# tatsy/opengl-raytracer

Measured on AMD Instinct MI355X. Metric: Mrays/s at 1920x1080, 8 bounces, higher is better.
Workload: dtype f32

## Files before the change

### opengl-raytracer_amd/csrc/pt_kernel.hip.h

```cpp
#pragma once
#include <hip/hip_runtime.h>
#include <stdint.h>

#include <type_traits>
#include "trav_asm.hip.h"
#include "scan_asm.hip.h"
#include "texture.hip.h"
#include "maps.hip.h"
#include "environment.hip.h"

namespace glrtx {

constexpr int kBlockThreads = 256;
constexpr int kTile = 16;
constexpr int REF_ABSENT = INT32_MIN;
constexpr int REF_FIN = INT32_MIN;
constexpr int kMaxLdsMaterials = 256;
constexpr int kMaxLdsLights = 64;
constexpr int kTopForks = 128;

constexpr float PT_EPS = 1.0e-4f;
constexpr float PT_INFTY = 1.0e8f;
constexpr float PT_PI = 3.14159274101257324f;
constexpr float PT_2PI = 6.28318548202514648f;
// ... 486 lines not shown
    }
    asm volatile(
        "s_mov_b64 %[entry], exec\n\t"
        "s_mov_b64 %[act], exec\n\t"
        GLRTX_ASM_SET_VBASE
        "v_bfrev_b32 v[GLRTX_VB+11], 1\n\t"
        GLRTX_REP(GLRTX_STEPS_PER_TRIP, GLRTX_TRAV_STEP_ASM_LANE)
        "99:\n\t"
        "s_mov_b64 exec, %[entry]"
        : [th] "+&v"(T.h.t), [tri] "+&v"(T.h.tri), [hu] "+&v"(T.h.u), [hv] "+&v"(T.h.v), [cur] "+&v"(T.cur), [sp] "+&v"(T.sp),
          [entry] "=&s"(s_entry), [act] "=&s"(s_act), [leaf] "=&s"(s_leaf), [bl] "=&s"(s_bl), [br] "=&s"(s_br), [pop] "=&s"(s_pop), [tmp] "=&s"(s_tmp) GLRTX_TS_OPERANDS
        : [ox] "v"(T.ox), [oy] "v"(T.oy), [oz] "v"(T.oz), [dx] "v"(T.dx), [dy] "v"(T.dy), [dz] "v"(T.dz), [ix] "v"(T.ix), [iy] "v"(T.iy), [iz] "v"(T.iz),
          [sd] "v"(T.stop_d), [stk] "v"(stk), [base] "s"(sc.nodes0), [bias] "s"(sc.node_bias), [eps] "s"(PT_EPS)
        : "vcc", "scc", "memory", GLRTX_ASM_VCLOBBERS GLRTX_TS_CLOBBERS);
}

struct TravLoop {
    unsigned long long act, uns;
    int pos, cnt;
    unsigned flags;
    unsigned rid, nr;
    float4 co, cd;
    float ix, iy, iz, lim;
};
#define GLRTX_LOOP_OUT \
    [th] "+&v"(T.h.t), [tri] "+&v"(T.h.tri), [hu] "+&v"(T.h.u), [hv] "+&v"(T.h.v), [cur] "+&v"(T.cur), [sp] "+&v"(T.sp), \
    [ox] "+&v"(T.ox), [oy] "+&v"(T.oy), [oz] "+&v"(T.oz), [dx] "+&v"(T.dx), [dy] "+&v"(T.dy), [dz] "+&v"(T.dz), [ix] "+&v"(T.ix), [iy] "+&v"(T.iy), [iz] "+&v"(T.iz), \
    [sd] "+&v"(T.stop_d), [rid] "+&v"(L.rid), [nr] "+&v"(L.nr), [act] "+&s"(L.act), [uns] "+&s"(L.uns), [pos] "+&s"(L.pos), \
    [entry] "=&s"(s_entry), [was] "=&s"(s_was), [leaf] "=&s"(s_leaf), [bl] "=&s"(s_bl), [br] "=&s"(s_br), [pop] "=&s"(s_pop), [tmp] "=&s"(s_tmp), \
    [n] "=&s"(s_n), [take] "=&s"(s_take), [why] "=&s"(why)
#define GLRTX_LOOP_IN \
    [cox] "v"(L.co.x), [coy] "v"(L.co.y), [coz] "v"(L.co.z), [cow] "v"(L.co.w), [cdx] "v"(L.cd.x), [cdy] "v"(L.cd.y), [cdz] "v"(L.cd.z), [cdw] "v"(L.cd.w), \
    [cix] "v"(L.ix), [ciy] "v"(L.iy), [ciz] "v"(L.iz), [clim] "v"(L.lim), [stk] "v"(stk), [cnt] "s"(cnt), [flags] "s"(flags), [rmin] "s"(rmin), [smax] "s"(smax), \
    [hbase] "s"(hbase), [lb] "s"(lb), [eps] "s"(PT_EPS)
template <int FETCH>
DEV int trav_loop_asm(const DevScene &sc, int *stack, Trav &T, TravLoop &L, int rmin, int smax, const void *hbase, unsigned lb, unsigned rk) {
    unsigned long long s_entry, s_was, s_leaf, s_bl, s_br, s_pop, s_tmp;
    int s_n, s_take, why;
    const unsigned stk = (unsigned)(uintptr_t)stack;
    static_assert(kBlockThreads * 8 == 1 << 11 && REF_FIN == INT32_MIN, "see trav_steps_asm");
    const int cnt = __builtin_amdgcn_readfirstlane(L.cnt);
    const unsigned flags = (unsigned)__builtin_amdgcn_readfirstlane((int)L.flags);
    rmin = __builtin_amdgcn_readfirstlane(rmin);
    smax = __builtin_amdgcn_readfirstlane(smax);
    const unsigned par16 = (threadIdx.x & 1u) << 4;
    const unsigned bias_e = sc.node_bias + par16, bias_o = sc.node_bias + 16u - par16;
    if constexpr ((FETCH & kWgwfCompact) != 0) {
        static_assert((FETCH & ~kWgwfCompact) == 0, "the compact layout has the one-record-per-lane fetch only");
        asm volatile(GLRTX_TRAV_LOOP_ASM(GLRTX_REP(GLRTX_STEPS_PER_TRIP, GLRTX_TRAV_STEP_ASM_COMPACT), "v[GLRTX_VB+22]", "0")
                     : GLRTX_LOOP_OUT
                     : GLRTX_LOOP_IN, [cbase] "s"(sc.cnodes), [rk] "s"(rk)
                     : "vcc", "scc", "memory", GLRTX_ASM_VCLOBBERS_COMPACT);
    } else if constexpr (FETCH == 2) {
        asm volatile(GLRTX_TRAV_LOOP_ASM(GLRTX_REP(GLRTX_STEPS_PER_TRIP_HALF, GLRTX_TRAV_STEP_ASM_PAIR GLRTX_TRAV_STEP_ASM_LANE), "v[GLRTX_VB+11]", "%[root]")
                     : GLRTX_LOOP_OUT
                     : GLRTX_LOOP_IN, [root] "s"(sc.root_ref), [base] "s"(sc.nodes0), [bias] "s"(sc.node_bias), [odd] "s"(0xAAAAAAAAAAAAAAAAull), [biase] "v"(bias_e), [biaso] "v"(bias_o)
                     : "vcc", "scc", "memory", GLRTX_ASM_VCLOBBERS_PAIR);
    } else if constexpr (FETCH == 1) {
        asm volatile(GLRTX_TRAV_LOOP_ASM(GLRTX_REP(GLRTX_STEPS_PER_TRIP, GLRTX_TRAV_STEP_ASM_PAIR), "v[GLRTX_VB+11]", "%[root]")
                     : GLRTX_LOOP_OUT
                     : GLRTX_LOOP_IN, [root] "s"(sc.root_ref), [base] "s"(sc.nodes0), [odd] "s"(0xAAAAAAAAAAAAAAAAull), [biase] "v"(bias_e), [biaso] "v"(bias_o)
                     : "vcc", "scc", "memory", GLRTX_ASM_VCLOBBERS_PAIR);
    } else {
        static_assert(FETCH == 0, "node fetch: 0 lane, 1 pair, 2 alternating, kWgwfCompact");
        asm volatile(GLRTX_TRAV_LOOP_ASM(GLRTX_REP(GLRTX_STEPS_PER_TRIP, GLRTX_TRAV_STEP_ASM_LANE), "v[GLRTX_VB+11]", "%[root]")
                     : GLRTX_LOOP_OUT
                     : GLRTX_LOOP_IN, [root] "s"(sc.root_ref), [base] "s"(sc.nodes0), [bias] "s"(sc.node_bias)
                     : "vcc", "scc", "memory", GLRTX_ASM_VCLOBBERS);
    }
    (void)rk; (void)bias_e; (void)bias_o;
    return why;
}

template <bool CLOSEST>
DEV void tri_test(Hit &h, int t, float ox, float oy, float oz, float dx, float dy, float dz, float v0x, float v0y, float v0z, float e1x,
                  float e1y, float e1z, float e2x, float e2y, float e2z, float tmin = PT_EPS) {
    const float tx = ox - v0x, ty = oy - v0y, tz = oz - v0z;
    const float px = dy * e2z - dz * e2y;
    const float py = dz * e2x - dx * e2z;
    const float pz = dx * e2y - dy * e2x;
    const float det = dot3(e1x, e1y, e1z, px, py, pz);
    const float U = dot3(tx, ty, tz, px, py, pz);
    const float inv = rcp_newton(det);
    const float u = U * inv;
    const bool ok_u = !(-PT_EPS < det && det < PT_EPS) && !(u < 0.0f || 1.0f < u);
    if (!__any(ok_u)) return;
    const float qx = ty * e1z - tz * e1y;
    const float qy = tz * e1x - tx * e1z;
    const float qz = tx * e1y - ty * e1x;
    const float V = dot3(dx, dy, dz, qx, qy, qz);
    const float v = V * inv;
    const bool ok_v = ok_u && !(v < 0.0f || 1.0f < inv * (U + V));
    if (!__any(ok_v)) return;
    const float tt = dot3(e2x, e2y, e2z, qx, qy, qz) * inv;
    const bool hit = ok_v && !(tmin >= tt);
// ... 1443 lines not shown
#define GLRTX_PRIO_SHADE 0
#endif
#ifndef GLRTX_WGWF_WAVES
#define GLRTX_WGWF_WAVES 4
#endif

#ifdef GLRTX_PHASE_STATS
__device__ unsigned long long g_phase_cycles[8];
__device__ uint4 g_trip_log[16][64];
#define PH_STAMP(var) const unsigned long long var = __builtin_amdgcn_s_memtime()
#define PH_ADD(i, t0, t1) do { if (threadIdx.x == 0) atomicAdd(&g_phase_cycles[i], (t1) - (t0)); } while (0)
#else
#define PH_STAMP(var)
#define PH_ADD(i, t0, t1)
#endif

#ifdef GLRTX_RAY_LOG
struct RayLog { float4 *rays; uint2 *trips; unsigned long long cap_rays; unsigned cap_trips; unsigned on; };
__device__ RayLog g_ray_log;
__device__ unsigned long long g_ray_log_n;
__device__ unsigned g_ray_log_trips;
#endif

DEV int wgwf_suspend_max();

#if defined(GLRTX_CXX_STEP) || defined(GLRTX_TRAV_STATS) || defined(GLRTX_PHASE_STATS) || defined(GLRTX_STEP_TIMING) || defined(GLRTX_RAY_LOG) || defined(GLRTX_CXX_LOOP)
#define GLRTX_TRAV_LOOP_CXX
#endif
template <bool VINE, int FETCH>
DEV void wg_traverse_phase(const KernelArgs &a, const WfArgs &w, const float4 *root, int *stack, const float4 *rq, int n_rays,
                           unsigned *ray_head, unsigned *light_bits, unsigned long long &rays, float4 *suspend_area) {
    const int lane = threadIdx.x & 63;
    const uint2 *ranks = reinterpret_cast<const uint2 *>(light_bits + kWgPathsMax / 32);
    if (VINE) {
        for (;;) {
            int base = 0;
            if (lane == 0) base = (int)atomicAdd(ray_head, 64u);
            base = __builtin_amdgcn_readfirstlane(base);
            if (base >= n_rays) break;
            float4 o = make_float4(0.f, 0.f, 0.f, __uint_as_float(WF_INVALID)), d = o;
            if (base + lane < n_rays) { o = ld_stream(&rq[2 * (size_t)(base + lane)]); d = ld_stream(&rq[2 * (size_t)(base + lane) + 1]); }
            const unsigned r = __float_as_uint(o.w);
            const bool shadow = (r & 1u) != 0u;
            const Hit h = trav_scan<true>(a.sc, o.x, o.y, o.z, d.x, d.y, d.z, r != WF_INVALID, shadow ? shadow_limit(d.w, a.sc.shadow_limited) : PT_INFTY,
                                          shadow ? d.w : -__builtin_inff());
            if (r != WF_INVALID) {
                rays++;
                if (r & 1u) { if (nee_accepted(d.w, h.t, h.tri >= 0)) atomicOr(&light_bits[r >> 6], 1u << ((r >> 1) & 31u)); }
                else st_stream(w.H(r >> 1), make_float4(h.t, __int_as_float(h.tri), h.u, h.v));
            }
        }
        return;
    }
    [[maybe_unused]] const unsigned long long lt_mask = (1ull << lane) - 1ull;
    const float4 none = make_float4(0.f, 0.f, 0.f, __uint_as_float(WF_INVALID));
    float4 cur_o = none, cur_d = none;
    float cur_ix = 0.f, cur_iy = 0.f, cur_iz = 0.f;
    [[maybe_unused]] int cur_pos = 0;
    int cur_cnt = 0;
#ifndef GLRTX_TRAV_LOOP_CXX
    float cur_lim = PT_INFTY;
#endif
    auto fetch = [&](float4 &o, float4 &d) -> int {
        int base = 0;
        if (lane == 0) base = (int)atomicAdd(ray_head, 64u);
        base = __builtin_amdgcn_readfirstlane(base);
        int cnt = n_rays - base;
        cnt = cnt < 0 ? 0 : (cnt > 64 ? 64 : cnt);
        if (lane < cnt) {
            o = ld_stream(&rq[2 * (size_t)(base + lane)]);
            d = ld_stream(&rq[2 * (size_t)(base + lane) + 1]);
            cur_ix = frcp(d.x); cur_iy = frcp(d.y); cur_iz = frcp(d.z);
            const bool shadow = (__float_as_uint(o.w) & 1u) != 0u;
            float t0;
            if (a.sc.root_boxed && !box_pass(root[0], root[1], o.x, o.y, o.z, cur_ix, cur_iy, cur_iz, shadow ? shadow_limit(d.w, a.sc.shadow_limited) : PT_INFTY, t0))
                d.w = __uint_as_float(__float_as_uint(d.w) | 0x80000000u);
#ifndef GLRTX_TRAV_LOOP_CXX
            cur_lim = shadow ? shadow_limit(__builtin_fabsf(d.w), a.sc.shadow_limited) : PT_INFTY;
#endif
        }
        return cnt;
    };
    cur_cnt = fetch(cur_o, cur_d);
    bool exhausted = cur_cnt == 0;
    const bool fetched_any = cur_cnt > 0;
    bool active = false;
    bool unsaved = false;
    unsigned rid = 0;
    Trav T;
    T.cur = 0; T.sp = 0;
    T.h.t = PT_INFTY; T.h.tri = -1; T.h.u = 0.f; T.h.v = 0.f;
#ifdef GLRTX_STEP_TIMING
    StepTiming step_timing;
#endif
    float4 *const susp = suspend_area + (size_t)kSuspendF4 * threadIdx.x;
    {
        const float4 s3 = susp[3];
        if (s3.z != 0.0f) {
            const float4 s0 = susp[0], s1 = susp[1], s2 = susp[2];
            susp[3] = make_float4(0.f, 0.f, 0.f, 0.f);
            T.ox = s0.x; T.oy = s0.y; T.oz = s0.z;
            rid = __float_as_uint(w.H(__float_as_uint(s0.w) >> 1)->y);
// ... 11 lines not shown
#ifdef GLRTX_FAULT_INJECT
            if (fault_dropped) active = false;
#endif
        }
    }
    auto save_hit = [&]() {
        const unsigned id = rid >> 1;
        if (rid & 1u) {
            if (nee_accepted(T.stop_d, T.h.t, T.h.tri >= 0)) atomicOr(&light_bits[id >> 5], 1u << (id & 31u));
        } else *w.H(id) = make_float4(T.h.t, __int_as_float(T.h.tri), T.h.u, T.h.v);
        unsaved = false;
    };
#ifndef GLRTX_TRAV_LOOP_CXX
    static_assert(WF_INVALID == 0xFFFFFFFFu, "trav_asm.hip.h compares a ray id with the inline constant -1");
    {
        TravLoop L;
        L.act = __ballot(active); L.uns = 0ull;
        L.pos = 0; L.cnt = cur_cnt;
        L.flags = exhausted ? 1u : 0u;
        L.rid = rid; L.nr = 0u;
        const void *const hbase = w.H(0u);
        const unsigned lb = (unsigned)(uintptr_t)light_bits;
        const int smax = wgwf_suspend_max();
        int why;
        for (;;) {
            L.co = cur_o; L.cd = cur_d; L.ix = cur_ix; L.iy = cur_iy; L.iz = cur_iz; L.lim = cur_lim;
            why = trav_loop_asm<FETCH>(a.sc, stack, T, L, w.refill_min, smax, hbase, lb, (unsigned)(uintptr_t)ranks);
            if (why != 1) break;
            cur_cnt = cur_cnt == 64 ? fetch(cur_o, cur_d) : 0;
            L.pos = 0; L.cnt = cur_cnt;
            L.flags = cur_cnt == 0 ? (1u | 2u | (fetched_any ? 4u : 0u)) : 2u;
        }
        rid = L.rid;
        rays += L.nr;
        active = ((L.act >> lane) & 1ull) != 0ull;
        unsaved = ((L.uns >> lane) & 1ull) != 0ull;
        if (why == 2 && active) {
            susp[0] = make_float4(T.ox, T.oy, T.oz, __uint_as_float(rid));
            susp[1] = make_float4(T.dx, T.dy, T.dz, T.stop_d);
            susp[2] = make_float4(T.h.t, __int_as_float(T.h.tri), T.h.u, T.h.v);
            susp[3] = make_float4(__int_as_float(T.cur), __int_as_float(T.sp), 1.0f, 0.f);
            float mark = kHitSuspended, zero = 0.f;
            asm volatile("" : "+v"(mark), "+v"(zero));
            *w.H(rid >> 1) = make_float4(mark, zero, zero, zero);
            active = false;
        }
    }
#else
#ifdef GLRTX_PHASE_STATS
    unsigned long long ph_refill = 0ull, ph_refills = 0ull, ph_step = 0ull;
#endif
    for (;;) {
        unsigned long long idle = __ballot(!active);
        if ((int)__popcll(idle) >= w.refill_min || idle == ~0ull) {
#ifdef GLRTX_PHASE_STATS
            const unsigned long long rf0 = __builtin_amdgcn_s_memtime();
#endif
            while (idle != 0ull && !exhausted) {
                if (cur_pos >= cur_cnt) {
                    cur_cnt = cur_cnt == 64 ? fetch(cur_o, cur_d) : 0;
                    cur_pos = 0;
                    if (cur_cnt == 0) { exhausted = true; break; }
                }
                const int n = __popcll(idle);
                const int avail = cur_cnt - cur_pos;
                const int take = n < avail ? n : avail;
                const int rank = __popcll(idle & lt_mask);
                const int src = (cur_pos + rank) & 63;
                const float ox = __shfl(cur_o.x, src), oy = __shfl(cur_o.y, src), oz = __shfl(cur_o.z, src);
                const unsigned new_rid = (unsigned)__shfl((int)__float_as_uint(cur_o.w), src);
                const float dx = __shfl(cur_d.x, src), dy = __shfl(cur_d.y, src), dz = __shfl(cur_d.z, src);
                const float dist_m = __shfl(cur_d.w, src);
                const float ix = __shfl(cur_ix, src), iy = __shfl(cur_iy, src), iz = __shfl(cur_iz, src);
                if (!active && rank < take) {
                    if (unsaved) save_hit();
                    rid = new_rid;
                    if (rid != WF_INVALID) {
                        rays++;
                        const bool shadow = (rid & 1u) != 0u;
                        const float dist = __builtin_fabsf(dist_m);
                        T.ox = ox; T.oy = oy; T.oz = oz; T.dx = dx; T.dy = dy; T.dz = dz; T.ix = ix; T.iy = iy; T.iz = iz;
                        T.h.t = shadow ? shadow_limit(dist, a.sc.shadow_limited) : PT_INFTY; T.h.tri = -1; T.h.u = 0.f; T.h.v = 0.f;
                        T.stop_d = shadow ? dist : -__builtin_inff();
                        T.sp = 0;
                        T.cur = (FETCH & kWgwfCompact) ? 0 : a.sc.root_ref;
#ifdef GLRTX_TRAV_STATS
                        T.iters = 0;
#endif
                        active = (__float_as_uint(dist_m) & 0x80000000u) == 0u;
                        unsaved = !active;
                    }
                }
                cur_pos += take;
                idle = __ballot(!active);
            }
#ifdef GLRTX_PHASE_STATS
            ph_refill += __builtin_amdgcn_s_memtime() - rf0; ph_refills += 1ull;
#endif
        }
        if (!__any(active)) {
            if (exhausted) break;
            continue;
        }
        if (exhausted && fetched_any) {
            const unsigned long long ma = __ballot(active);
            const int suspend_max = wgwf_suspend_max();
            if (__ballot(active && (rid & 1u) != 0u) == 0ull && (int)__popcll(ma) <= suspend_max) {
                if (active) {
                    susp[0] = make_float4(T.ox, T.oy, T.oz, __uint_as_float(rid));
                    susp[1] = make_float4(T.dx, T.dy, T.dz, T.stop_d);
                    susp[2] = make_float4(T.h.t, __int_as_float(T.h.tri), T.h.u, T.h.v);
                    susp[3] = make_float4(__int_as_float(T.cur), __int_as_float(T.sp), 1.0f, 0.f);
// ... 301 lines not shown
                unsigned tid = threadIdx.x;
                asm volatile("" : "+v"(tid));
                if (tid < kWgPathsMax / 32) light_bits[tid] = 0u;
            }
            const int nr = (int)ctl[2 + cur], np = (int)ctl[4 + cur];
            float4 *rq_w = rayQ + 2 * ((size_t)cur * 2 * kWgPaths + nr);
            const WgwfKernArgs *kt = wgwf_kernargs();
            const unsigned new_base = kt->w.set_base(cur, (int)blockIdx.x) + (unsigned)np;
            for (int k = threadIdx.x; k < got; k += kBlockThreads) {
                int id = tile0 * 64 + k;
                if (ADAPT) {
                    const int g = tile0 + (k >> 6), n_active = (int)*kt->adapt_count;
                    const int frame = g / n_active;
                    id = frame * kt->w.total + kt->adapt_list[g - frame * n_active] * 64 + (k & 63);
                }
                float4 ro = make_float4(0.f, 0.f, 0.f, __uint_as_float(WF_INVALID)), rd = ro;
                const bool go = wf_generate_one(kt->a, kt->w, lds_cam, id, new_base + (unsigned)k, ro, rd);
                rq_w[2 * k] = ro;
                rq_w[2 * k + 1] = rd;
                (void)go;
            }
            __syncthreads();
            if (tid_topup == 0u) { ctl[2 + cur] = (unsigned)(nr + got); ctl[4 + cur] = (unsigned)(np + got); ctl[1] = 0u; }
        }
        __syncthreads();
        PH_STAMP(pg1);
        PH_ADD(0, pg0, pg1);
        const int n_rays = (int)ctl[2 + cur], n_paths = (int)ctl[4 + cur];
        if (n_paths == 0) {
            if (look_again) continue;
            break;
        }
        const float4 *rq = rayQ + 2 * ((size_t)cur * 2 * kWgPaths);

#ifdef GLRTX_RAY_LOG
        if (g_ray_log.on) {
            if (threadIdx.x == 0) {
                const unsigned long long base = atomicAdd(&g_ray_log_n, (unsigned long long)n_rays);
                ctl[9] = 0u;
                if (base + (unsigned long long)n_rays <= g_ray_log.cap_rays) {
                    const unsigned t = atomicAdd(&g_ray_log_trips, 1u);
                    if (t < g_ray_log.cap_trips) { g_ray_log.trips[t] = make_uint2((unsigned)base, (unsigned)n_rays); ctl[8] = (unsigned)base; ctl[9] = 1u; }
                }
            }
            __syncthreads();
            if (ctl[9]) {
                float4 *dst = g_ray_log.rays + 2 * (size_t)ctl[8];
                for (int i = threadIdx.x; i < 2 * n_rays; i += kBlockThreads) dst[i] = rq[i];
            }
            __syncthreads();
        }
#endif
        PH_STAMP(pt0);
        __builtin_amdgcn_s_setprio(GLRTX_PRIO_TRAVERSE);
        wg_traverse_phase<VINE, NODE_FETCH>(a, w, lds_root, stack, rq, n_rays, &ctl[1], light_bits, rays, rayQ + kWgSuspendAt);
        __builtin_amdgcn_s_setprio(GLRTX_PRIO_SHADE);
        PH_STAMP(pt1);
        __syncthreads();
        PH_STAMP(pt2);
        PH_ADD(1, pt0, pt1);
        PH_ADD(2, pt1, pt2);

        const WgwfKernArgs *ks = wgwf_kernargs();
        wg_shade_phase<VOL, TEX, MAPS>(ks->a, ks->w, lds_mats, lds_cam, light_bits, n_paths, rayQ + 2 * ((size_t)(cur ^ 1) * 2 * kWgPaths),
                            &ctl[2 + (cur ^ 1)], &ctl[4 + (cur ^ 1)], ks->w.set_base(cur, (int)blockIdx.x), ks->w.set_base(cur ^ 1, (int)blockIdx.x), rays, &ctl[10]);
        PH_STAMP(ps1);
        __syncthreads();
        PH_STAMP(ps2);
        PH_ADD(3, pt2, ps1);
        PH_ADD(4, ps1, ps2);
#ifdef GLRTX_PHASE_STATS
        if (threadIdx.x == 0 && (blockIdx.x & 63) == 0 && blockIdx.x / 64 < 16) {
            uint4 *lg = g_trip_log[blockIdx.x / 64];
            const unsigned n = lg[0].x + 1u;
            if (n < 64u) { lg[n] = make_uint4((unsigned)n_rays, (unsigned)n_paths, (unsigned)(pt2 - pt0), (unsigned)(ps2 - pt2)); lg[0].x = n; }
        }
#endif
        unsigned tid_end = threadIdx.x;
// ... 31 lines not shown
__global__ __launch_bounds__(kBlockThreads, GLRTX_WGWF_WAVES) void pt_replay_traverse(const KernelArgs a, const WfArgs w, unsigned *work_counter, float4 *wg_queues,
                                                                                      const float4 *log, const uint2 *trips, int n_trips) {
    extern __shared__ __attribute__((aligned(16))) unsigned char lds_raw[];
    const int mat_f4 = a.sc.lds_head_f4;
    unsigned char *pl = lds_raw + (size_t)mat_f4 * sizeof(float4);
    int *stack = reinterpret_cast<int *>(pl) + 2 * threadIdx.x;
    pl += (size_t)2 * a.sc.stack_entries * kBlockThreads * sizeof(int);
    unsigned *ctl = reinterpret_cast<unsigned *>(pl);
    float4 *lds_root = reinterpret_cast<float4 *>(pl + kWgCtlWords * sizeof(unsigned));
    unsigned *light_bits = reinterpret_cast<unsigned *>(pl + kWgCtlWords * sizeof(unsigned) + 32 + kCamFloatsPadded * 4 + kLdsSeeds * 8);
    if (threadIdx.x == 64) lds_root[0] = a.sc.root_lo;
    if (threadIdx.x == 65) lds_root[1] = a.sc.root_hi;
    float4 *rayQ = wg_queues + (size_t)blockIdx.x * kWgQueueF4;
    rayQ[kWgSuspendAt + (size_t)kSuspendF4 * threadIdx.x + 3] = make_float4(0.f, 0.f, 0.f, 0.f);
    unsigned long long rays = 0;
    __syncthreads();
    for (;;) {
        if (threadIdx.x == 0) { ctl[0] = atomicAdd(work_counter, 1u); ctl[1] = 0u; }
        if (threadIdx.x < kWgPathsMax / 32) light_bits[threadIdx.x] = 0u;
        __syncthreads();
        const unsigned t = ctl[0];
        if (t >= (unsigned)n_trips) break;
        const uint2 tr = trips[t];
        __builtin_amdgcn_s_setprio(GLRTX_PRIO_TRAVERSE);
        wg_traverse_phase<false, FETCH>(a, w, lds_root, stack, log + 2 * (size_t)tr.x, (int)tr.y, &ctl[1], light_bits, rays, rayQ + kWgSuspendAt);
        __builtin_amdgcn_s_setprio(GLRTX_PRIO_SHADE);
        __syncthreads();
    }
    flush_rays<true>(a, rays);
}
#endif


constexpr float kAdaptLumFloor = 1e-3f;
constexpr int kAdaptCompactThreads = 1024;

__global__ __launch_bounds__(256) void adaptive_select_kernel(const float4 *accum, const float4 *half, int pitch_f4, int width, int rows, int tiles8_x, int n_tiles,
                                                              float threshold, int min_samples, unsigned char *mask, float *tile_err) {
    const int tile = blockIdx.x * 4 + (threadIdx.x >> 6), k = threadIdx.x & 63;
    if (tile >= n_tiles) return;
    const int x = (tile % tiles8_x) * 8 + (k & 7), y = (tile / tiles8_x) * 8 + (k >> 3);
    const bool in = x < width && y < rows;
    float d = 0.0f;
    bool force = false;
    if (in) {
        const size_t at = (size_t)y * pitch_f4 + x;
        const float4 c = ld_stream(&accum[at]), h = ld_stream(&half[at]);
        force = c.w < (float)min_samples || h.w == 0.0f;
// ... 136 lines not shown
```

### opengl-raytracer_amd/csrc/trav_asm.hip.h

```cpp
#pragma once

#ifndef GLRTX_STEPS_PER_TRIP
#define GLRTX_STEPS_PER_TRIP 6
#endif
#ifndef GLRTX_ASM_VBASE
#define GLRTX_ASM_VBASE 96
#endif
static_assert(GLRTX_STEPS_PER_TRIP % 2 == 0, "the alternating form of the node fetch unrolls steps in pairs");
#define GLRTX_STEPS_PER_TRIP_HALF_(n) GLRTX_HALF_##n
#define GLRTX_HALF_2 1
#define GLRTX_HALF_4 2
#define GLRTX_HALF_6 3
#define GLRTX_HALF_8 4
#define GLRTX_STEPS_PER_TRIP_HALF_X(n) GLRTX_STEPS_PER_TRIP_HALF_(n)
#define GLRTX_STEPS_PER_TRIP_HALF GLRTX_STEPS_PER_TRIP_HALF_X(GLRTX_STEPS_PER_TRIP)
#define GLRTX_STR_(x) #x
#define GLRTX_STR(x) GLRTX_STR_(x)
#define GLRTX_ASM_SET_VBASE ".set GLRTX_VB, " GLRTX_STR(GLRTX_ASM_VBASE) "\n\t"
#if GLRTX_ASM_VBASE == 96
#define GLRTX_ASM_VCLOBBERS "v96", "v97", "v98", "v99", "v100", "v101", "v102", "v103", "v104", "v105", "v106", "v107", "v108", "v109", "v110", "v111", "v112", "v113", "v114", "v115", "v116", "v117"
#define GLRTX_ASM_VCLOBBERS_PAIR GLRTX_ASM_VCLOBBERS, "v118", "v119"
#define GLRTX_ASM_VCLOBBERS_COMPACT GLRTX_ASM_VCLOBBERS_PAIR
#elif GLRTX_ASM_VBASE == 72
#define GLRTX_ASM_VCLOBBERS "v72", "v73", "v74", "v75", "v76", "v77", "v78", "v79", "v80", "v81", "v82", "v83", "v84", "v85", "v86", "v87", "v88", "v89", "v90", "v91", "v92", "v93"
// ... 340 lines not shown
    "s_or_b64 %[pop], %[pop], vcc\n\t"                                                                                                                \
    "21:\n\t"                                                                                                                                          \
    "s_mov_b64 exec, %[pop]\n\t"                                         \
    "s_cbranch_execz 30f\n\t"                                                                                                                          \
    "10:\n\t"                                                                                                                                          \
    "v_cmp_ne_u32 vcc, 0, %[sp]\n\t"                                                                                                                   \
    "v_cndmask_b32 %[cur], " FIN ", %[cur], vcc\n\t"                                                                \
    "s_and_b64 exec, exec, vcc\n\t"                                                                                                                    \
    "s_cbranch_execz 30f\n\t"                                                                                                                          \
    "v_add_u32 %[sp], -1, %[sp]\n\t"                                                                                                                   \
    "v_lshl_add_u32 v[GLRTX_VB+15], %[sp], 11, %[stk]\n\t"                                                                                                       \
    "ds_read_b64 v[GLRTX_VB+16:GLRTX_VB+17], v[GLRTX_VB+15]\n\t"                                                                                                  \
    "s_waitcnt lgkmcnt(0)\n\t"                                                                                                                         \
    "v_mov_b32 %[cur], v[GLRTX_VB+17]\n\t"                                                                                                                       \
    "v_cmp_gt_f32 vcc, v[GLRTX_VB+16], %[th]\n\t"                                                                                                                \
    "s_and_b64 exec, exec, vcc\n\t"                                                                                                                    \
    "s_cbranch_execnz 10b\n\t"                                                                                                                         \
    "30:\n\t"                                                                                                                                          \
    "s_mov_b64 exec, %[act]\n\t"                                                                                  \
    GLRTX_TS_END                                                                                                                       \
    "v_cmpx_ne_u32_e64 %[act], %[cur], " FIN "\n\t"                                                                             \
    "s_cbranch_execz 99f\n\t"

#define GLRTX_TRAV_LOOP_ASM(STEPS, FIN, ROOT) \
    "s_mov_b64 %[entry], exec\n\t" \
    "s_mov_b64 exec, -1\n\t" \
    GLRTX_ASM_SET_VBASE \
    "v_bfrev_b32 " FIN ", 1\n\t" \
    "s_bitcmp1_b32 %[flags], 1\n\t"                                      \
    "s_cbranch_scc1 72f\n\t" \
    "70:\n\t"                                                            \
    "s_cmp_eq_u64 %[act], 0\n\t" \
    "s_cbranch_scc1 72f\n\t" \
    "s_not_b64 %[tmp], %[act]\n\t" \
    "s_bcnt1_i32_b64 %[n], %[tmp]\n\t" \
    "s_cmp_ge_i32 %[n], %[rmin]\n\t" \
    "s_cbranch_scc0 79f\n\t" \
    "72:\n\t"                                                            \
    "s_not_b64 vcc, %[act]\n\t"                                          \
    "s_cbranch_scc0 78f\n\t" \
    "s_bitcmp1_b32 %[flags], 0\n\t" \
    "s_cbranch_scc1 78f\n\t" \
    "s_cmp_ge_i32 %[pos], %[cnt]\n\t" \
    "s_cbranch_scc1 97f\n\t"                                             \
    "s_bcnt1_i32_b64 %[n], vcc\n\t" \
    "s_sub_i32 %[take], %[cnt], %[pos]\n\t" \
    "s_min_i32 %[take], %[take], %[n]\n\t"                               \
    "v_mbcnt_lo_u32_b32 v[GLRTX_VB+14], vcc_lo, 0\n\t"                   \
    "v_mbcnt_hi_u32_b32 v[GLRTX_VB+14], vcc_hi, v[GLRTX_VB+14]\n\t" \
    "v_add_lshl_u32 v[GLRTX_VB+13], v[GLRTX_VB+14], %[pos], 2\n\t"       \
    "v_and_b32 v[GLRTX_VB+13], 0xfc, v[GLRTX_VB+13]\n\t" \
    "ds_bpermute_b32 v[GLRTX_VB+3], v[GLRTX_VB+13], %[cow]\n\t"          \
    "ds_bpermute_b32 v[GLRTX_VB+7], v[GLRTX_VB+13], %[cdw]\n\t" \
    "ds_bpermute_b32 v[GLRTX_VB+0], v[GLRTX_VB+13], %[cox]\n\t" \
    "ds_bpermute_b32 v[GLRTX_VB+1], v[GLRTX_VB+13], %[coy]\n\t" \
    "ds_bpermute_b32 v[GLRTX_VB+2], v[GLRTX_VB+13], %[coz]\n\t" \
    "ds_bpermute_b32 v[GLRTX_VB+4], v[GLRTX_VB+13], %[cdx]\n\t" \
    "ds_bpermute_b32 v[GLRTX_VB+5], v[GLRTX_VB+13], %[cdy]\n\t" \
    "ds_bpermute_b32 v[GLRTX_VB+6], v[GLRTX_VB+13], %[cdz]\n\t" \
    "ds_bpermute_b32 v[GLRTX_VB+8], v[GLRTX_VB+13], %[cix]\n\t" \
    "ds_bpermute_b32 v[GLRTX_VB+9], v[GLRTX_VB+13], %[ciy]\n\t" \
    "ds_bpermute_b32 v[GLRTX_VB+10], v[GLRTX_VB+13], %[ciz]\n\t" \
    "ds_bpermute_b32 v[GLRTX_VB+12], v[GLRTX_VB+13], %[clim]\n\t" \
    "v_cmp_gt_i32_e64 %[leaf], %[take], v[GLRTX_VB+14]\n\t" \
    "s_and_b64 %[leaf], %[leaf], vcc\n\t"                                \
    "s_and_b64 exec, %[leaf], %[uns]\n\t"                                \
    "s_cbranch_scc0 74f\n\t" \
    "s_mov_b64 %[br], exec\n\t" \
    "v_and_b32 v[GLRTX_VB+15], 1, %[rid]\n\t" \
    "v_cmp_eq_u32_e64 %[bl], 1, v[GLRTX_VB+15]\n\t"                      \
    "v_lshrrev_b32 v[GLRTX_VB+15], 1, %[rid]\n\t"                        \
    "s_andn2_b64 exec, exec, %[bl]\n\t"                                  \
    "s_cbranch_execz 73f\n\t"                                            \
    "v_lshlrev_b32 v[GLRTX_VB+20], 4, v[GLRTX_VB+15]\n\t" \
    "v_mov_b32 v[GLRTX_VB+16], %[th]\n\t" \
    "v_mov_b32 v[GLRTX_VB+17], %[tri]\n\t" \
    "v_mov_b32 v[GLRTX_VB+18], %[hu]\n\t" \
    "v_mov_b32 v[GLRTX_VB+19], %[hv]\n\t" \
    "global_store_dwordx4 v[GLRTX_VB+20], v[GLRTX_VB+16:GLRTX_VB+19], %[hbase]\n\t" \
    "73:\n\t" \
    "s_and_b64 exec, %[br], %[bl]\n\t"                                   \
    "v_sub_f32 v[GLRTX_VB+21], %[sd], %[th]\n\t" \
    "v_cmp_lt_f32_e64 %[bl], |v[GLRTX_VB+21]|, %[eps]\n\t" \
    "v_cmp_le_i32_e64 %[br], 0, %[tri]\n\t" \
    "s_and_b64 %[bl], %[bl], %[br]\n\t" \
    "s_and_b64 exec, exec, %[bl]\n\t" \
    "v_lshlrev_b32_e64 v[GLRTX_VB+21], v[GLRTX_VB+15], 1\n\t"            \
    "v_lshrrev_b32 v[GLRTX_VB+14], 5, v[GLRTX_VB+15]\n\t" \
    "v_lshl_add_u32 v[GLRTX_VB+14], v[GLRTX_VB+14], 2, %[lb]\n\t" \
    "ds_or_b32 v[GLRTX_VB+14], v[GLRTX_VB+21]\n\t" \
    "74:\n\t" \
    "s_andn2_b64 %[uns], %[uns], %[leaf]\n\t" \
    "s_mov_b64 exec, %[leaf]\n\t"                                        \
    "s_waitcnt lgkmcnt(0)\n\t" \
    "v_mov_b32 %[rid], v[GLRTX_VB+3]\n\t" \
    "v_cmpx_ne_u32_e64 %[bl], -1, v[GLRTX_VB+3]\n\t"                     \
    "v_add_u32 %[nr], 1, %[nr]\n\t" \
    "v_mov_b32 %[ox], v[GLRTX_VB+0]\n\t" \
    "v_mov_b32 %[oy], v[GLRTX_VB+1]\n\t" \
    "v_mov_b32 %[oz], v[GLRTX_VB+2]\n\t" \
    "v_mov_b32 %[dx], v[GLRTX_VB+4]\n\t" \
    "v_mov_b32 %[dy], v[GLRTX_VB+5]\n\t" \
    "v_mov_b32 %[dz], v[GLRTX_VB+6]\n\t" \
    "v_mov_b32 %[ix], v[GLRTX_VB+8]\n\t" \
    "v_mov_b32 %[iy], v[GLRTX_VB+9]\n\t" \
    "v_mov_b32 %[iz], v[GLRTX_VB+10]\n\t" \
    "v_mov_b32 %[th], v[GLRTX_VB+12]\n\t"                                \
    "v_mov_b32 %[tri], -1\n\t" \
    "v_mov_b32 %[hu], 0\n\t" \
    "v_mov_b32 %[hv], 0\n\t" \
    "v_mov_b32 %[sp], 0\n\t" \
    "v_mov_b32 %[cur], " ROOT "\n\t" \
    "v_and_b32 v[GLRTX_VB+15], 1, %[rid]\n\t" \
    "v_cmp_eq_u32_e64 %[bl], 1, v[GLRTX_VB+15]\n\t"                      \
    "v_and_b32 v[GLRTX_VB+16], 0x7fffffff, v[GLRTX_VB+7]\n\t" \
    "v_mov_b32 v[GLRTX_VB+17], 0xff800000\n\t" \
    "v_cndmask_b32_e64 %[sd], v[GLRTX_VB+17], v[GLRTX_VB+16], %[bl]\n\t" \
    "v_cmp_le_i32_e64 %[bl], 0, v[GLRTX_VB+7]\n\t"                       \
    "s_or_b64 %[act], %[act], %[bl]\n\t" \
    "s_andn2_b64 %[bl], exec, %[bl]\n\t"                                 \
    "s_or_b64 %[uns], %[uns], %[bl]\n\t" \
    "s_add_i32 %[pos], %[pos], %[take]\n\t" \
    "s_mov_b64 exec, -1\n\t" \
    "s_branch 72b\n\t" \
    "78:\n\t"                                                            \
    "s_cmp_eq_u64 %[act], 0\n\t" \
    "s_cbranch_scc0 79f\n\t" \
    "s_bitcmp1_b32 %[flags], 0\n\t" \
    "s_cbranch_scc1 96f\n\t"                                             \
    "s_branch 70b\n\t" \
    "79:\n\t"                                                            \
    "s_bitcmp1_b32 %[flags], 2\n\t" \
    "s_cbranch_scc0 80f\n\t" \
    "s_mov_b64 exec, %[act]\n\t" \
    "v_and_b32 v[GLRTX_VB+15], 1, %[rid]\n\t" \
    "v_cmp_eq_u32_e64 %[bl], 1, v[GLRTX_VB+15]\n\t" \
    "s_cmp_eq_u64 %[bl], 0\n\t"                                          \
    "s_cbranch_scc0 80f\n\t" \
    "s_bcnt1_i32_b64 %[n], %[act]\n\t" \
    "s_cmp_le_i32 %[n], %[smax]\n\t" \
    "s_cbranch_scc1 98f\n\t" \
    "80:\n\t"                                                            \
    "s_mov_b64 exec, %[act]\n\t" \
    "s_mov_b64 %[was], %[act]\n\t" \
// ... 29 lines not shown
```

Measured before the change: 10630.

## Precompute per-ray reciprocals, root box test and first root step in a prepare pass

Adds a wg_prepare_rays pass that, once rays are queued, computes reciprocal directions, the shadow limit, the root-box cull and the first root-node child test for every ray. It writes these to a side buffer, and the traversal refill then loads them instead of recomputing. The inline-asm refill now takes the precomputed start node and pushes the far child onto the stack when both root children are hit. The cost is an extra global write and read per ray and two more bpermutes per refill, in exchange for skipping the root visit during traversal and moving the per-ray setup off the divergent traversal path.

```diff
diff --git a/opengl-raytracer_amd/csrc/pt_kernel.hip.h b/opengl-raytracer_amd/csrc/pt_kernel.hip.h
--- a/opengl-raytracer_amd/csrc/pt_kernel.hip.h
+++ b/opengl-raytracer_amd/csrc/pt_kernel.hip.h
@@ -532,6 +532,7 @@
     unsigned rid, nr;
     float4 co, cd;
     float ix, iy, iz, lim;
+    float cur0, t0;
 };
 #define GLRTX_LOOP_OUT \
     [th] "+&v"(T.h.t), [tri] "+&v"(T.h.tri), [hu] "+&v"(T.h.u), [hv] "+&v"(T.h.v), [cur] "+&v"(T.cur), [sp] "+&v"(T.sp), \
@@ -541,10 +542,11 @@
     [n] "=&s"(s_n), [take] "=&s"(s_take), [why] "=&s"(why)
 #define GLRTX_LOOP_IN \
     [cox] "v"(L.co.x), [coy] "v"(L.co.y), [coz] "v"(L.co.z), [cow] "v"(L.co.w), [cdx] "v"(L.cd.x), [cdy] "v"(L.cd.y), [cdz] "v"(L.cd.z), [cdw] "v"(L.cd.w), \
-    [cix] "v"(L.ix), [ciy] "v"(L.iy), [ciz] "v"(L.iz), [clim] "v"(L.lim), [stk] "v"(stk), [cnt] "s"(cnt), [flags] "s"(flags), [rmin] "s"(rmin), [smax] "s"(smax), \
+    [cix] "v"(L.ix), [ciy] "v"(L.iy), [ciz] "v"(L.iz), [clim] "v"(L.lim), [ccur] "v"(L.cur0), [ct0] "v"(L.t0), [stk] "v"(stk), [cnt] "s"(cnt), [flags] "s"(flags), [rmin] "s"(rmin), [smax] "s"(smax), \
     [hbase] "s"(hbase), [lb] "s"(lb), [eps] "s"(PT_EPS)
+#ifndef GLRTX_STEP_TIMING
 template <int FETCH>
-DEV int trav_loop_asm(const DevScene &sc, int *stack, Trav &T, TravLoop &L, int rmin, int smax, const void *hbase, unsigned lb, unsigned rk) {
+DEV int trav_loop_asm(const DevScene &sc, int *stack, Trav &T, TravLoop &L, int rmin, int smax, const void *hbase, unsigned lb, unsigned rk, int rootl) {
     unsigned long long s_entry, s_was, s_leaf, s_bl, s_br, s_pop, s_tmp;
     int s_n, s_take, why;
     const unsigned stk = (unsigned)(uintptr_t)stack;
@@ -553,34 +555,36 @@
     const unsigned flags = (unsigned)__builtin_amdgcn_readfirstlane((int)L.flags);
     rmin = __builtin_amdgcn_readfirstlane(rmin);
     smax = __builtin_amdgcn_readfirstlane(smax);
+    rootl = __builtin_amdgcn_readfirstlane(rootl);
     const unsigned par16 = (threadIdx.x & 1u) << 4;
     const unsigned bias_e = sc.node_bias + par16, bias_o = sc.node_bias + 16u - par16;
     if constexpr ((FETCH & kWgwfCompact) != 0) {
         static_assert((FETCH & ~kWgwfCompact) == 0, "the compact layout has the one-record-per-lane fetch only");
-        asm volatile(GLRTX_TRAV_LOOP_ASM(GLRTX_REP(GLRTX_STEPS_PER_TRIP, GLRTX_TRAV_STEP_ASM_COMPACT), "v[GLRTX_VB+22]", "0")
+        asm volatile(GLRTX_TRAV_LOOP_ASM(GLRTX_REP(GLRTX_STEPS_PER_TRIP, GLRTX_TRAV_STEP_ASM_COMPACT), "v[GLRTX_VB+22]", "1")
                      : GLRTX_LOOP_OUT
                      : GLRTX_LOOP_IN, [cbase] "s"(sc.cnodes), [rk] "s"(rk)
                      : "vcc", "scc", "memory", GLRTX_ASM_VCLOBBERS_COMPACT);
     } else if constexpr (FETCH == 2) {
-        asm volatile(GLRTX_TRAV_LOOP_ASM(GLRTX_REP(GLRTX_STEPS_PER_TRIP_HALF, GLRTX_TRAV_STEP_ASM_PAIR GLRTX_TRAV_STEP_ASM_LANE), "v[GLRTX_VB+11]", "%[root]")
+        asm volatile(GLRTX_TRAV_LOOP_ASM(GLRTX_REP(GLRTX_STEPS_PER_TRIP_HALF, GLRTX_TRAV_STEP_ASM_PAIR GLRTX_TRAV_STEP_ASM_LANE), "v[GLRTX_VB+11]", "%[rootl]")
                      : GLRTX_LOOP_OUT
-                     : GLRTX_LOOP_IN, [root] "s"(sc.root_ref), [base] "s"(sc.nodes0), [bias] "s"(sc.node_bias), [odd] "s"(0xAAAAAAAAAAAAAAAAull), [biase] "v"(bias_e), [biaso] "v"(bias_o)
+                     : GLRTX_LOOP_IN, [rootl] "s"(rootl), [base] "s"(sc.nodes0), [bias] "s"(sc.node_bias), [odd] "s"(0xAAAAAAAAAAAAAAAAull), [biase] "v"(bias_e), [biaso] "v"(bias_o)
                      : "vcc", "scc", "memory", GLRTX_ASM_VCLOBBERS_PAIR);
     } else if constexpr (FETCH == 1) {
-        asm volatile(GLRTX_TRAV_LOOP_ASM(GLRTX_REP(GLRTX_STEPS_PER_TRIP, GLRTX_TRAV_STEP_ASM_PAIR), "v[GLRTX_VB+11]", "%[root]")
+        asm volatile(GLRTX_TRAV_LOOP_ASM(GLRTX_REP(GLRTX_STEPS_PER_TRIP, GLRTX_TRAV_STEP_ASM_PAIR), "v[GLRTX_VB+11]", "%[rootl]")
                      : GLRTX_LOOP_OUT
-                     : GLRTX_LOOP_IN, [root] "s"(sc.root_ref), [base] "s"(sc.nodes0), [odd] "s"(0xAAAAAAAAAAAAAAAAull), [biase] "v"(bias_e), [biaso] "v"(bias_o)
+                     : GLRTX_LOOP_IN, [rootl] "s"(rootl), [base] "s"(sc.nodes0), [odd] "s"(0xAAAAAAAAAAAAAAAAull), [biase] "v"(bias_e), [biaso] "v"(bias_o)
                      : "vcc", "scc", "memory", GLRTX_ASM_VCLOBBERS_PAIR);
     } else {
         static_assert(FETCH == 0, "node fetch: 0 lane, 1 pair, 2 alternating, kWgwfCompact");
-        asm volatile(GLRTX_TRAV_LOOP_ASM(GLRTX_REP(GLRTX_STEPS_PER_TRIP, GLRTX_TRAV_STEP_ASM_LANE), "v[GLRTX_VB+11]", "%[root]")
+        asm volatile(GLRTX_TRAV_LOOP_ASM(GLRTX_REP(GLRTX_STEPS_PER_TRIP, GLRTX_TRAV_STEP_ASM_LANE), "v[GLRTX_VB+11]", "%[rootl]")
                      : GLRTX_LOOP_OUT
-                     : GLRTX_LOOP_IN, [root] "s"(sc.root_ref), [base] "s"(sc.nodes0), [bias] "s"(sc.node_bias)
+                     : GLRTX_LOOP_IN, [rootl] "s"(rootl), [base] "s"(sc.nodes0), [bias] "s"(sc.node_bias)
                      : "vcc", "scc", "memory", GLRTX_ASM_VCLOBBERS);
     }
-    (void)rk; (void)bias_e; (void)bias_o;
+    (void)rk; (void)bias_e; (void)bias_o; (void)rootl;
     return why;
 }
+#endif
 
 template <bool CLOSEST>
 DEV void tri_test(Hit &h, int t, float ox, float oy, float oz, float dx, float dy, float dz, float v0x, float v0y, float v0z, float e1x,
@@ -2070,13 +2074,60 @@
 __device__ unsigned g_ray_log_trips;
 #endif
 
+constexpr unsigned kNoStackedChild = 0x7FC00000u;
+template <int FETCH>
+DEV int wgwf_root_left(const DevScene &sc) {
+    if constexpr ((FETCH & kWgwfCompact) != 0) return 1;
+    else return __float_as_int(reinterpret_cast<const float4 *>(reinterpret_cast<const char *>(sc.nodes0) + ((unsigned)sc.root_ref * 64u + sc.node_bias))->w);
+}
+template <int FETCH>
+DEV void wg_prepare_rays(const DevScene &sc, const float4 *root, const uint2 *ranks, const float4 *rq, float4 *prep, int n_rays) {
+    constexpr bool CP = (FETCH & kWgwfCompact) != 0;
+    const int root_ref = CP ? 0 : sc.root_ref;
+    const bool root_step = sc.root_boxed != 0 && (CP ? (ranks[0].x & 1u) != 0u : root_ref >= 0);
+    float4 A = make_float4(0.f, 0.f, 0.f, 0.f), B = A, C = A, D = A;
+    int l = REF_FIN, r = REF_FIN;
+    if (root_step) {
+        if constexpr (CP) {
+            A = sc.cnodes[0]; B = sc.cnodes[1]; C = sc.cnodes[2];
+            D = make_float4(A.w, B.w, C.w, 0.f);
+            l = wgwf_root_left<FETCH>(sc); r = l + 1;
+        } else {
+            const float4 *N = reinterpret_cast<const float4 *>(reinterpret_cast<const char *>(sc.nodes0) + ((unsigned)root_ref * 64u + sc.node_bias));
+            A = N[0]; B = N[1]; C = N[2]; D = N[3];
+            asm volatile("" : "+v"(C.w), "+v"(D.w));
+            l = __float_as_int(A.w); r = __float_as_int(B.w);
+        }
+    }
+    for (int i = threadIdx.x; i < n_rays; i += kBlockThreads) {
+        const float4 o = rq[2 * (size_t)i], d = rq[2 * (size_t)i + 1];
+        const unsigned rid = __float_as_uint(o.w);
+        if (rid == WF_INVALID) continue;
+        const bool shadow = (rid & 1u) != 0u;
+        const float ix = frcp(d.x), iy = frcp(d.y), iz = frcp(d.z);
+        const float lim = shadow ? shadow_limit(d.w, sc.shadow_limited) : PT_INFTY;
+        int cur0 = root_ref;
+        float t0 = __uint_as_float(kNoStackedChild), t;
+        if (sc.root_boxed && !box_pass(root[0], root[1], o.x, o.y, o.z, ix, iy, iz, lim, t)) cur0 = REF_FIN;
+        else if (root_step) {
+            float t0r;
+            const bool pl = box_pass(A, B, o.x, o.y, o.z, ix, iy, iz, lim, t);
+            const bool pr = box_pass(C, D, o.x, o.y, o.z, ix, iy, iz, lim, t0r);
+            cur0 = pr ? r : (pl ? l : REF_FIN);
+            if (pl && pr) t0 = t;
+        }
+        prep[2 * (size_t)i] = make_float4(ix, iy, iz, lim);
+        prep[2 * (size_t)i + 1] = make_float4(__int_as_float(cur0), t0, shadow ? d.w : -__builtin_inff(), 0.f);
+    }
+}
+
 DEV int wgwf_suspend_max();
 
 #if defined(GLRTX_CXX_STEP) || defined(GLRTX_TRAV_STATS) || defined(GLRTX_PHASE_STATS) || defined(GLRTX_STEP_TIMING) || defined(GLRTX_RAY_LOG) || defined(GLRTX_CXX_LOOP)
 #define GLRTX_TRAV_LOOP_CXX
 #endif
 template <bool VINE, int FETCH>
-DEV void wg_traverse_phase(const KernelArgs &a, const WfArgs &w, const float4 *root, int *stack, const float4 *rq, int n_rays,
+DEV void wg_traverse_phase(const KernelArgs &a, const WfArgs &w, int *stack, const float4 *rq, const float4 *prep, int n_rays,
                            unsigned *ray_head, unsigned *light_bits, unsigned long long &rays, float4 *suspend_area) {
     const int lane = threadIdx.x & 63;
     const uint2 *ranks = reinterpret_cast<const uint2 *>(light_bits + kWgPathsMax / 32);
@@ -2103,12 +2154,10 @@
     [[maybe_unused]] const unsigned long long lt_mask = (1ull << lane) - 1ull;
     const float4 none = make_float4(0.f, 0.f, 0.f, __uint_as_float(WF_INVALID));
     float4 cur_o = none, cur_d = none;
-    float cur_ix = 0.f, cur_iy = 0.f, cur_iz = 0.f;
+    float4 cur_p = none;
+    float cur_c0 = 0.f, cur_t0 = 0.f;
     [[maybe_unused]] int cur_pos = 0;
     int cur_cnt = 0;
-#ifndef GLRTX_TRAV_LOOP_CXX
-    float cur_lim = PT_INFTY;
-#endif
     auto fetch = [&](float4 &o, float4 &d) -> int {
         int base = 0;
         if (lane == 0) base = (int)atomicAdd(ray_head, 64u);
@@ -2118,14 +2167,9 @@
         if (lane < cnt) {
             o = ld_stream(&rq[2 * (size_t)(base + lane)]);
             d = ld_stream(&rq[2 * (size_t)(base + lane) + 1]);
-            cur_ix = frcp(d.x); cur_iy = frcp(d.y); cur_iz = frcp(d.z);
-            const bool shadow = (__float_as_uint(o.w) & 1u) != 0u;
-            float t0;
-            if (a.sc.root_boxed && !box_pass(root[0], root[1], o.x, o.y, o.z, cur_ix, cur_iy, cur_iz, shadow ? shadow_limit(d.w, a.sc.shadow_limited) : PT_INFTY, t0))
-                d.w = __uint_as_float(__float_as_uint(d.w) | 0x80000000u);
-#ifndef GLRTX_TRAV_LOOP_CXX
-            cur_lim = shadow ? shadow_limit(__builtin_fabsf(d.w), a.sc.shadow_limited) : PT_INFTY;
-#endif
+            cur_p = ld_stream(&prep[2 * (size_t)(base + lane)]);
+            const float4 q = ld_stream(&prep[2 * (size_t)(base + lane) + 1]);
+            cur_c0 = q.x; cur_t0 = q.y; d.w = q.z;
         }
         return cnt;
     };
@@ -2183,10 +2227,11 @@
         const void *const hbase = w.H(0u);
         const unsigned lb = (unsigned)(uintptr_t)light_bits;
         const int smax = wgwf_suspend_max();
+        const int rootl = wgwf_root_left<FETCH>(a.sc);
         int why;
         for (;;) {
-            L.co = cur_o; L.cd = cur_d; L.ix = cur_ix; L.iy = cur_iy; L.iz = cur_iz; L.lim = cur_lim;
-            why = trav_loop_asm<FETCH>(a.sc, stack, T, L, w.refill_min, smax, hbase, lb, (unsigned)(uintptr_t)ranks);
+            L.co = cur_o; L.cd = cur_d; L.ix = cur_p.x; L.iy = cur_p.y; L.iz = cur_p.z; L.lim = cur_p.w; L.cur0 = cur_c0; L.t0 = cur_t0;
+            why = trav_loop_asm<FETCH>(a.sc, stack, T, L, w.refill_min, smax, hbase, lb, (unsigned)(uintptr_t)ranks, rootl);
             if (why != 1) break;
             cur_cnt = cur_cnt == 64 ? fetch(cur_o, cur_d) : 0;
             L.pos = 0; L.cnt = cur_cnt;
@@ -2231,24 +2276,28 @@
                 const float ox = __shfl(cur_o.x, src), oy = __shfl(cur_o.y, src), oz = __shfl(cur_o.z, src);
                 const unsigned new_rid = (unsigned)__shfl((int)__float_as_uint(cur_o.w), src);
                 const float dx = __shfl(cur_d.x, src), dy = __shfl(cur_d.y, src), dz = __shfl(cur_d.z, src);
-                const float dist_m = __shfl(cur_d.w, src);
-                const float ix = __shfl(cur_ix, src), iy = __shfl(cur_iy, src), iz = __shfl(cur_iz, src);
+                const float stop_d = __shfl(cur_d.w, src);
+                const float ix = __shfl(cur_p.x, src), iy = __shfl(cur_p.y, src), iz = __shfl(cur_p.z, src), lim = __shfl(cur_p.w, src);
+                const int c0 = __shfl(__float_as_int(cur_c0), src);
+                const float t0 = __shfl(cur_t0, src);
                 if (!active && rank < take) {
                     if (unsaved) save_hit();
                     rid = new_rid;
                     if (rid != WF_INVALID) {
                         rays++;
-                        const bool shadow = (rid & 1u) != 0u;
-                        const float dist = __builtin_fabsf(dist_m);
                         T.ox = ox; T.oy = oy; T.oz = oz; T.dx = dx; T.dy = dy; T.dz = dz; T.ix = ix; T.iy = iy; T.iz = iz;
-                        T.h.t = shadow ? shadow_limit(dist, a.sc.shadow_limited) : PT_INFTY; T.h.tri = -1; T.h.u = 0.f; T.h.v = 0.f;
-                        T.stop_d = shadow ? dist : -__builtin_inff();
+                        T.h.t = lim; T.h.tri = -1; T.h.u = 0.f; T.h.v = 0.f;
+                        T.stop_d = stop_d;
+                        T.cur = c0;
                         T.sp = 0;
-                        T.cur = (FETCH & kWgwfCompact) ? 0 : a.sc.root_ref;
+                        if (t0 == t0) {
+                            reinterpret_cast<int2 *>(stack)[0] = make_int2(__float_as_int(t0), wgwf_root_left<FETCH>(a.sc));
+                            T.sp = 1;
+                        }
 #ifdef GLRTX_TRAV_STATS
                         T.iters = 0;
 #endif
-                        active = (__float_as_uint(dist_m) & 0x80000000u) == 0u;
+                        active = c0 != REF_FIN;
                         unsaved = !active;
                     }
                 }
@@ -2596,6 +2645,9 @@
             }
             __syncthreads();
             if (tid_topup == 0u) { ctl[2 + cur] = (unsigned)(nr + got); ctl[4 + cur] = (unsigned)(np + got); ctl[1] = 0u; }
+            if (!VINE)
+                wg_prepare_rays<NODE_FETCH>(kt->a.sc, lds_root, reinterpret_cast<const uint2 *>(light_bits + kWgPathsMax / 32), rayQ + 2 * ((size_t)cur * 2 * kWgPaths),
+                                            rayQ + 2 * ((size_t)(cur ^ 1) * 2 * kWgPaths), nr + got);
         }
         __syncthreads();
         PH_STAMP(pg1);
@@ -2627,7 +2679,7 @@
 #endif
         PH_STAMP(pt0);
         __builtin_amdgcn_s_setprio(GLRTX_PRIO_TRAVERSE);
-        wg_traverse_phase<VINE, NODE_FETCH>(a, w, lds_root, stack, rq, n_rays, &ctl[1], light_bits, rays, rayQ + kWgSuspendAt);
+        wg_traverse_phase<VINE, NODE_FETCH>(a, w, stack, rq, rayQ + 2 * ((size_t)(cur ^ 1) * 2 * kWgPaths), n_rays, &ctl[1], light_bits, rays, rayQ + kWgSuspendAt);
         __builtin_amdgcn_s_setprio(GLRTX_PRIO_SHADE);
         PH_STAMP(pt1);
         __syncthreads();
@@ -2705,8 +2757,10 @@
         const unsigned t = ctl[0];
         if (t >= (unsigned)n_trips) break;
         const uint2 tr = trips[t];
+        wg_prepare_rays<FETCH>(a.sc, lds_root, nullptr, log + 2 * (size_t)tr.x, rayQ, (int)tr.y);
+        __syncthreads();
         __builtin_amdgcn_s_setprio(GLRTX_PRIO_TRAVERSE);
-        wg_traverse_phase<false, FETCH>(a, w, lds_root, stack, log + 2 * (size_t)tr.x, (int)tr.y, &ctl[1], light_bits, rays, rayQ + kWgSuspendAt);
+        wg_traverse_phase<false, FETCH>(a, w, stack, log + 2 * (size_t)tr.x, rayQ, (int)tr.y, &ctl[1], light_bits, rays, rayQ + kWgSuspendAt);
         __builtin_amdgcn_s_setprio(GLRTX_PRIO_SHADE);
         __syncthreads();
     }
diff --git a/opengl-raytracer_amd/csrc/trav_asm.hip.h b/opengl-raytracer_amd/csrc/trav_asm.hip.h
--- a/opengl-raytracer_amd/csrc/trav_asm.hip.h
+++ b/opengl-raytracer_amd/csrc/trav_asm.hip.h
@@ -386,7 +386,7 @@
     "v_cmpx_ne_u32_e64 %[act], %[cur], " FIN "\n\t"                                                                             \
     "s_cbranch_execz 99f\n\t"
 
-#define GLRTX_TRAV_LOOP_ASM(STEPS, FIN, ROOT) \
+#define GLRTX_TRAV_LOOP_ASM(STEPS, FIN, ROOTL) \
     "s_mov_b64 %[entry], exec\n\t" \
     "s_mov_b64 exec, -1\n\t" \
     GLRTX_ASM_SET_VBASE \
@@ -414,8 +414,10 @@
     "v_mbcnt_hi_u32_b32 v[GLRTX_VB+14], vcc_hi, v[GLRTX_VB+14]\n\t" \
     "v_add_lshl_u32 v[GLRTX_VB+13], v[GLRTX_VB+14], %[pos], 2\n\t"       \
     "v_and_b32 v[GLRTX_VB+13], 0xfc, v[GLRTX_VB+13]\n\t" \
+    "v_cmp_gt_i32_e64 %[leaf], %[take], v[GLRTX_VB+14]\n\t" \
+    "s_and_b64 %[leaf], %[leaf], vcc\n\t"                                \
     "ds_bpermute_b32 v[GLRTX_VB+3], v[GLRTX_VB+13], %[cow]\n\t"          \
-    "ds_bpermute_b32 v[GLRTX_VB+7], v[GLRTX_VB+13], %[cdw]\n\t" \
+    "ds_bpermute_b32 v[GLRTX_VB+7], v[GLRTX_VB+13], %[cdw]\n\t"          \
     "ds_bpermute_b32 v[GLRTX_VB+0], v[GLRTX_VB+13], %[cox]\n\t" \
     "ds_bpermute_b32 v[GLRTX_VB+1], v[GLRTX_VB+13], %[coy]\n\t" \
     "ds_bpermute_b32 v[GLRTX_VB+2], v[GLRTX_VB+13], %[coz]\n\t" \
@@ -426,8 +428,8 @@
     "ds_bpermute_b32 v[GLRTX_VB+9], v[GLRTX_VB+13], %[ciy]\n\t" \
     "ds_bpermute_b32 v[GLRTX_VB+10], v[GLRTX_VB+13], %[ciz]\n\t" \
     "ds_bpermute_b32 v[GLRTX_VB+12], v[GLRTX_VB+13], %[clim]\n\t" \
-    "v_cmp_gt_i32_e64 %[leaf], %[take], v[GLRTX_VB+14]\n\t" \
-    "s_and_b64 %[leaf], %[leaf], vcc\n\t"                                \
+    "ds_bpermute_b32 v[GLRTX_VB+14], v[GLRTX_VB+13], %[ct0]\n\t"         \
+    "ds_bpermute_b32 v[GLRTX_VB+13], v[GLRTX_VB+13], %[ccur]\n\t"        \
     "s_and_b64 exec, %[leaf], %[uns]\n\t"                                \
     "s_cbranch_scc0 74f\n\t" \
     "s_mov_b64 %[br], exec\n\t" \
@@ -450,9 +452,9 @@
     "s_and_b64 %[bl], %[bl], %[br]\n\t" \
     "s_and_b64 exec, exec, %[bl]\n\t" \
     "v_lshlrev_b32_e64 v[GLRTX_VB+21], v[GLRTX_VB+15], 1\n\t"            \
-    "v_lshrrev_b32 v[GLRTX_VB+14], 5, v[GLRTX_VB+15]\n\t" \
-    "v_lshl_add_u32 v[GLRTX_VB+14], v[GLRTX_VB+14], 2, %[lb]\n\t" \
-    "ds_or_b32 v[GLRTX_VB+14], v[GLRTX_VB+21]\n\t" \
+    "v_lshrrev_b32 v[GLRTX_VB+15], 5, v[GLRTX_VB+15]\n\t" \
+    "v_lshl_add_u32 v[GLRTX_VB+15], v[GLRTX_VB+15], 2, %[lb]\n\t" \
+    "ds_or_b32 v[GLRTX_VB+15], v[GLRTX_VB+21]\n\t" \
     "74:\n\t" \
     "s_andn2_b64 %[uns], %[uns], %[leaf]\n\t" \
     "s_mov_b64 exec, %[leaf]\n\t"                                        \
@@ -473,17 +475,17 @@
     "v_mov_b32 %[tri], -1\n\t" \
     "v_mov_b32 %[hu], 0\n\t" \
     "v_mov_b32 %[hv], 0\n\t" \
-    "v_mov_b32 %[sp], 0\n\t" \
-    "v_mov_b32 %[cur], " ROOT "\n\t" \
-    "v_and_b32 v[GLRTX_VB+15], 1, %[rid]\n\t" \
-    "v_cmp_eq_u32_e64 %[bl], 1, v[GLRTX_VB+15]\n\t"                      \
-    "v_and_b32 v[GLRTX_VB+16], 0x7fffffff, v[GLRTX_VB+7]\n\t" \
-    "v_mov_b32 v[GLRTX_VB+17], 0xff800000\n\t" \
-    "v_cndmask_b32_e64 %[sd], v[GLRTX_VB+17], v[GLRTX_VB+16], %[bl]\n\t" \
-    "v_cmp_le_i32_e64 %[bl], 0, v[GLRTX_VB+7]\n\t"                       \
+    "v_mov_b32 %[sd], v[GLRTX_VB+7]\n\t" \
+    "v_mov_b32 %[cur], v[GLRTX_VB+13]\n\t"                               \
+    "v_cmp_ne_u32_e64 %[bl], v[GLRTX_VB+13], " FIN "\n\t"                \
     "s_or_b64 %[act], %[act], %[bl]\n\t" \
     "s_andn2_b64 %[bl], exec, %[bl]\n\t"                                 \
     "s_or_b64 %[uns], %[uns], %[bl]\n\t" \
+    "v_cmp_o_f32_e64 %[br], v[GLRTX_VB+14], v[GLRTX_VB+14]\n\t"          \
+    "v_cndmask_b32_e64 %[sp], 0, 1, %[br]\n\t" \
+    "v_mov_b32 v[GLRTX_VB+15], " ROOTL "\n\t" \
+    "s_mov_b64 exec, %[br]\n\t" \
+    "ds_write_b64 %[stk], v[GLRTX_VB+14:GLRTX_VB+15]\n\t"                \
     "s_add_i32 %[pos], %[pos], %[take]\n\t" \
     "s_mov_b64 exec, -1\n\t" \
     "s_branch 72b\n\t" \
```

Result: slower. 9483 (-10.8%).
